# mlaprise/mfrec

Measured on NVIDIA B200. Metric: rating_updates_per_s, higher is better.
Workload: dtype f32

## Files before the change

### include/mfrec_b200.h

```cpp
#ifndef MFREC_B200_H
#define MFREC_B200_H

#include <stdint.h>

#ifdef __cplusplus
extern "C" {
#endif

#define MFREC_B200_ABI_VERSION 6

typedef enum mfrec_status {
    MFREC_OK = 0,
    MFREC_ERR_BAD_ARG = -1,
    MFREC_ERR_INDEX = -2,
    MFREC_ERR_OOM = -3,
    MFREC_ERR_CUDA = -4,
    MFREC_ERR_UNSUPPORTED = -5
} mfrec_status;

typedef struct mfrec_ctx mfrec_ctx;
typedef struct mfrec_ratings mfrec_ratings;
typedef struct mfrec_model mfrec_model;

enum { MFREC_KERNEL_LINEAR = 0,
       MFREC_KERNEL_LOGISTIC = 1    };

enum { MFREC_FUNK_WITHOUT_BIAS = 0,
       MFREC_FUNK_WITH_BIAS = 1,
       MFREC_FUNK_WITH_BIAS_DEV = 2   };

enum { MFREC_PRED_GD_RATING = 0,
       MFREC_PRED_GD_RATING_BIAS = 1,
// ... 117 lines not shown
int mfrec_bias_stats(mfrec_ctx *ctx, const int32_t *ratings_index, const double *ratings,
                     int64_t nnz, int32_t ni, int32_t nu, double K2, double K3, double *mu_out,
                     double *items_bias, double *users_bias);

int mfrec_train_als_wrmf(mfrec_ctx *ctx, int nbr_epochs, int k, double *u, double *v,
                         const int32_t *users_row, int64_t n_users_row, const int32_t *users_col,
                         const int32_t *items_row, int64_t n_items_row, const int32_t *items_col,
                         int32_t nbr_users, int32_t nbr_items, int c_pos, double reg);

int mfrec_train_als_wrmf_multi(const int32_t *devices, int n_shards, int nbr_epochs, int k,
                               double *u, double *v,
                               const int32_t *users_row, int64_t n_users_row, const int32_t *users_col,
                               const int32_t *items_row, int64_t n_items_row, const int32_t *items_col,
                               int32_t nbr_users, int32_t nbr_items, int c_pos, double reg);


int mfrec_ratings_pack(mfrec_ctx *ctx, const int32_t *ratings_index, const void *ratings,
                       int ratings_are_f32, int is_device, int64_t nnz, int32_t ni, int32_t nu,
                       const int64_t *item_degree, const mfrec_opts *opts,
                       mfrec_ratings **out);
void mfrec_ratings_destroy(mfrec_ratings *r);
int mfrec_ratings_info(const mfrec_ratings *r, int64_t info[8]);
int mfrec_ratings_quad_types(const mfrec_ratings *r, int64_t counts[4]);
int mfrec_ratings_perm(mfrec_ctx *ctx, const mfrec_ratings *r, int32_t *user_perm,
                       int32_t *item_perm);
int mfrec_ratings_order(mfrec_ctx *ctx, const mfrec_ratings *r, int64_t *order);
int mfrec_ratings_offsets(mfrec_ctx *ctx, const mfrec_ratings *r, int64_t *offsets,
                          int32_t *counts);
int mfrec_ratings_packed(mfrec_ctx *ctx, const mfrec_ratings *r, void *out);
int mfrec_ratings_copies(const mfrec_ratings *r, int32_t *vbase, int64_t counts[2]);
int mfrec_ratings_slab_items(const mfrec_ratings *r, int32_t slab, int32_t *begin, int32_t *end);

int mfrec_model_create(mfrec_ctx *ctx, const mfrec_ratings *layout, int k, int32_t ni,
                       int32_t nu, const double *u, const double *v, const double *items_bias,
                       const double *users_bias, mfrec_model **out);
int mfrec_model_read(mfrec_ctx *ctx, const mfrec_model *m, double *u, double *v,
                     double *items_bias, double *users_bias);
void mfrec_model_destroy(mfrec_model *m);
int mfrec_model_device_ptrs(const mfrec_model *m, void *ptrs[4], int64_t dims[3]);

int mfrec_sgd_epoch(mfrec_ctx *ctx, const mfrec_ratings *r, mfrec_model *m, int kernel,
                    double learning_rate, double K_users, double K_items, double K_bias,
                    int update_users, int update_items, int32_t slab, double *sq_err_out);

typedef struct mfrec_ring mfrec_ring;
int mfrec_ring_create(mfrec_ctx *ctx, const mfrec_ratings *r, mfrec_model *m, int rank, int world,
// ... 33 lines not shown
```

### mfrec_b200/_native.py

```python
import ctypes as C
import os
import threading

import numpy as np

_HERE = os.path.dirname(os.path.abspath(__file__))
LIB_PATH = os.environ.get("MFREC_B200_LIB") or os.path.join(_HERE, "libmfrec_b200.so")

OK = 0
ERR_BAD_ARG, ERR_INDEX, ERR_OOM, ERR_CUDA, ERR_UNSUPPORTED = -1, -2, -3, -4, -5

KERNEL_LINEAR, KERNEL_LOGISTIC = 0, 1
FUNK_WITHOUT_BIAS, FUNK_WITH_BIAS, FUNK_WITH_BIAS_DEV = 0, 1, 2
SCHED_STRATIFIED, SCHED_SEQUENTIAL = 0, 1
FOLD_USERS, FOLD_ITEMS = 0, 1

PREDICTORS = {
    "predict_rating": 0,
    "predict_rating_with_bias": 1,
    "predict_linear": 2,
    "predict_logistic": 3,
    "predict_linear_neg": 4,
    "predict_dot": 5,
}

EXPORTS = (
    "mfrec_abi_version", "mfrec_ctx_create", "mfrec_ctx_destroy", "mfrec_last_error",
    "mfrec_ctx_stream", "mfrec_ctx_sync", "mfrec_ctx_launch_count", "mfrec_train_kmf",
    "mfrec_train_funk", "mfrec_funk_loop_dev", "mfrec_funk_subloop", "mfrec_funk_predictor_subloop",
    "mfrec_train_funk_learned_bias", "mfrec_train_als_wrmf", "mfrec_predict_pairs", "mfrec_rmse_pairs", "mfrec_topn", "mfrec_topn_sweep",
    "mfrec_bias_stats", "mfrec_ratings_pack", "mfrec_ratings_destroy", "mfrec_ratings_info",
    "mfrec_ratings_quad_types", "mfrec_ratings_perm", "mfrec_ratings_order", "mfrec_ratings_offsets", "mfrec_ratings_packed",
    "mfrec_ratings_slab_items", "mfrec_model_create", "mfrec_model_read", "mfrec_model_destroy",
    "mfrec_model_device_ptrs", "mfrec_sgd_epoch", "mfrec_model_predict",
    "mfrec_ring_create", "mfrec_ring_destroy", "mfrec_ring_handle", "mfrec_ring_connect",
    "mfrec_ring_connect_local", "mfrec_ring_epochs", "mfrec_ring_epochs_one_device", "mfrec_ring_wait",
    "mfrec_ring_sync_model", "mfrec_model_topn", "mfrec_model_topn_sweep", "mfrec_ratings_copies",
    "mfrec_train_kmf_multi", "mfrec_fold_in_kmf", "mfrec_fold_in_funk", "mfrec_train_als_wrmf_multi",
)


class MfrecError(RuntimeError):

    def __init__(self, code, message):
        RuntimeError.__init__(self, "libmfrec_b200 error %d: %s" % (code, message))
        self.code = code


SPLIT_AUTO, SPLIT_ON, SPLIT_OFF = 0, 1, 2
STORAGE_F32, STORAGE_F16, STORAGE_BF16 = 0, 1, 2


class Opts(C.Structure):
    _fields_ = [("schedule", C.c_int32), ("row_blocks", C.c_int32), ("workers", C.c_int32),
                ("n_slabs", C.c_int32), ("keep_order", C.c_int32), ("k_hint", C.c_int32),
# ... 382 lines not shown
        _check(lib().mfrec_ratings_perm(self.ctx.handle, self._h, _ptr(up), _ptr(ip)), self.ctx.handle)
        return up, ip

    def order(self):
        out = np.zeros(self.packed_len, dtype=np.int64)
        _check(lib().mfrec_ratings_order(self.ctx.handle, self._h, _ptr(out)), self.ctx.handle)
        return out

    def offsets(self):
        off = np.zeros(self.n_buckets + 1, dtype=np.int64)
        cnt = np.zeros(self.n_buckets, dtype=np.int32)
        _check(lib().mfrec_ratings_offsets(self.ctx.handle, self._h, _ptr(off), _ptr(cnt)),
               self.ctx.handle)
        return off, cnt

    def packed(self):
        raw = np.zeros((self.packed_len, 3), dtype=np.int32)
        _check(lib().mfrec_ratings_packed(self.ctx.handle, self._h, _ptr(raw)), self.ctx.handle)
        return raw[:, 0].copy(), raw[:, 1].copy(), raw[:, 2].copy().view(np.float32)

    def quad_types(self):
        out = (C.c_int64 * 4)()
        _check(lib().mfrec_ratings_quad_types(self._h, out))
        return dict(generic=int(out[0]), chain=int(out[1]), clean=int(out[2]), independent=int(out[3]))

    def copies(self):
        vb = np.zeros(self.ni + 1, dtype=np.int32)
        cnt = (C.c_int64 * 2)()
        _check(lib().mfrec_ratings_copies(self._h, _ptr(vb), cnt))
        return vb, int(cnt[0]), int(cnt[1])

    def slab_items(self, slab):
        a, b = C.c_int32(), C.c_int32()
        _check(lib().mfrec_ratings_slab_items(self._h, C.c_int32(slab), C.byref(a), C.byref(b)))
        return a.value, b.value

    def replay_order(self, by_slab=False):
        order = self.order()
        off, cnt = self.offsets()
        B, W, G = self.B, self.W, self.G
        off = off[:-1].reshape(G, B, B, W * W)
        cnt = cnt.reshape(G, B, B, W * W)
        slabs = []
        for g in range(G):
            out = []
            for s in range(B):
                for rb in range(B):
# ... 181 lines not shown
```

### mfrec_b200/csrc/common.cuh

```cuda
#pragma once

#include <cuda_bf16.h>
#include <cuda_fp16.h>
#include <cuda_runtime.h>
#include <stdint.h>

#include <cstdarg>
#include <cstdio>
#include <future>
#include <memory>
#include <string>
#include <vector>

#include "mfrec_b200.h"

struct __align__(4) PackedRating {
    int32_t u;
    int32_t i;
    float r;
};
static_assert(sizeof(PackedRating) == 12, "rating triple must be 12 bytes");
constexpr int32_t kIdMask = 0x07ffffff;
constexpr int32_t kFlagAdjUser = 1 << 27;
constexpr int32_t kFlagStale = 1 << 28;
constexpr int32_t kFlagSameItem = 1 << 29;
constexpr int32_t kFlagPad = 1 << 30;
constexpr int kQuadShift = 28;
constexpr int kQuadGeneric = 0;
constexpr int kQuadChain = 1;
constexpr int kQuadClean = 2;
constexpr int kQuadIndep = 3;

struct mfrec_ctx {
    int device = 0;
    int sm_count = 0;
    size_t smem_optin = 0;
    size_t smem_per_sm = 0;
    int coop_launch = 0;
    cudaStream_t stream = nullptr;
    int64_t launches = 0;
    double *se_scratch = nullptr;
    size_t se_cap = 0;
    int32_t *ticks = nullptr;
    size_t ticks_cap = 0;
    cudaStream_t copy_stream = nullptr;
    cudaEvent_t values_ready = nullptr;
    struct {
        const double *u = nullptr, *v = nullptr, *ib = nullptr, *ub = nullptr;
        cudaEvent_t ready = nullptr;
    } staged;
    std::shared_future<int> values_enqueued, factors_enqueued;
    int refs = 1;
    std::shared_ptr<void> pack_host;
    std::shared_ptr<void> stager;
    std::string err;
};
void mfrec_ctx_retain(mfrec_ctx *ctx);
void mfrec_ctx_release(mfrec_ctx *ctx);

struct mfrec_ratings {
    mfrec_ctx *ctx = nullptr;
    int device = 0;
    int64_t nnz = 0;
    int32_t ni = 0, nu = 0;
    int B = 1, W = 1, G = 1;
    int storage = 0;
    int64_t n_buckets = 0;
    int64_t packed_len = 0;
    int32_t max_cb_items = 0;
    int64_t max_bucket = 0;
    float max_abs_rating = 0.f;
    int64_t quad_types[4] = {0, 0, 0, 0};
    int32_t ni_v = 0;
    int32_t n_hot = 0;
    int32_t *user_perm = nullptr;
    int32_t *item_perm = nullptr;
    int32_t *item_rows = nullptr;
    int32_t *item_vbase = nullptr;
    int32_t *vitem_src = nullptr;
    int32_t *hot_off = nullptr;
    int32_t *hot_rows = nullptr;
    int32_t *col_start = nullptr;
    PackedRating *packed = nullptr;
    int64_t *bucket_off = nullptr;
    int32_t *bucket_cnt = nullptr;
    int64_t *order = nullptr;
    std::vector<int32_t> h_row_start;
    std::vector<int32_t> h_col_start;
    std::vector<int32_t> h_vbase;
};

struct mfrec_model {
    mfrec_ctx *ctx = nullptr;
    int device = 0;
    int k = 0, kpad = 0;
// ... 22 lines not shown
            const int lu = __shfl_sync(full, level, pu < 0 ? lane : pu);
            const int li = __shfl_sync(full, level, pi < 0 ? lane : pi);
            int nl = 1;
            if (pu >= 0) nl = lu + 1;
            if (pi >= 0) nl = max(nl, li + 1);
            const bool changed = nl != level;
            level = nl;
            if (!__any_sync(full, changed)) break;
        }
    }
    lmax = __reduce_max_sync(full, live ? level : 0);
    return level;
}

__device__ __forceinline__ uint32_t smem_u32(const void *p) { return (uint32_t)__cvta_generic_to_shared(p); }
__device__ __forceinline__ void mbar_init(uint64_t *bar, uint32_t count)
{
    asm volatile("mbarrier.init.shared::cta.b64 [%0], %1;" ::"r"(smem_u32(bar)), "r"(count));
}
__device__ __forceinline__ void mbar_expect_tx(uint64_t *bar, uint32_t bytes)
{
    asm volatile("mbarrier.arrive.expect_tx.shared::cta.b64 _, [%0], %1;" ::"r"(smem_u32(bar)), "r"(bytes) : "memory");
}
__device__ __forceinline__ void mbar_wait(uint64_t *bar, uint32_t parity)
{
    asm volatile(
        "{\n"
        ".reg .pred p;\n"
        "WAIT_%=:\n"
        "mbarrier.try_wait.parity.shared::cta.b64 p, [%0], %1;\n"
        "@p bra DONE_%=;\n"
        "bra WAIT_%=;\n"
        "DONE_%=:\n"
        "}\n" ::"r"(smem_u32(bar)),
        "r"(parity)
        : "memory");
}
__device__ __forceinline__ void bulk_g2s(void *dst_smem, const void *src_gmem, uint32_t bytes, uint64_t *bar)
{
    asm volatile(
        "cp.async.bulk.shared::cluster.global.mbarrier::complete_tx::bytes [%0], [%1], %2, [%3];" ::"r"(smem_u32(dst_smem)),
        "l"(src_gmem), "r"(bytes), "r"(smem_u32(bar))
        : "memory");
}

__device__ __forceinline__ int ld_acquire_gpu(const int32_t *p)
{
// ... 136 lines not shown
```

### mfrec_b200/csrc/pack.cu

```cuda
#include <algorithm>
#include <cstring>
#include <cub/device/device_radix_sort.cuh>
#include <cub/device/device_scan.cuh>
#include <numeric>
#include <queue>

#include "common.cuh"
#include "partition.h"

namespace {

__global__ void degree_kernel(const int32_t *__restrict__ idx, int64_t nnz, int32_t ni, int32_t nu,
                              int32_t *__restrict__ deg_u, int32_t *__restrict__ deg_i,
                              int32_t *__restrict__ bad)
{
    const int64_t stride = (int64_t)gridDim.x * blockDim.x;
    for (int64_t n = (int64_t)blockIdx.x * blockDim.x + threadIdx.x; n < nnz; n += stride) {
        const int2 ui = reinterpret_cast<const int2 *>(idx)[n];
        if (ui.x < 0 || ui.x >= nu || ui.y < 0 || ui.y >= ni) {
            atomicOr(bad, 1);
            continue;
        }
        atomicAdd(&deg_u[ui.x], 1);
        atomicAdd(&deg_i[ui.y], 1);
// ... 123 lines not shown
    }
}

__global__ void max_abs_rating_kernel(const PackedRating *__restrict__ packed, int64_t n,
                                      int32_t *__restrict__ out_bits)
{
    int32_t mx = 0;
    const int64_t stride = (int64_t)gridDim.x * blockDim.x;
    for (int64_t j = (int64_t)blockIdx.x * blockDim.x + threadIdx.x; j < n; j += stride)
        mx = max(mx, __float_as_int(fabsf(packed[j].r)));
    for (int o = 16; o > 0; o >>= 1) mx = max(mx, __shfl_xor_sync(0xffffffffu, mx, o));
    if ((threadIdx.x & 31) == 0) atomicMax(out_bits, mx);
}

__global__ void fill_padding_kernel(PackedRating *__restrict__ packed, int64_t n)
{
    const int64_t stride = (int64_t)gridDim.x * blockDim.x;
    PackedRating pad;
    pad.u = 0; pad.i = kFlagPad; pad.r = 0.f;
    for (int64_t j = (int64_t)blockIdx.x * blockDim.x + threadIdx.x; j < n; j += stride) packed[j] = pad;
}

__global__ void quad_type_kernel(PackedRating *__restrict__ packed, int64_t n_quads,
                                 unsigned long long *__restrict__ type_count)
{
    const int64_t stride = (int64_t)gridDim.x * blockDim.x;
    int mine[4] = {0, 0, 0, 0};
    for (int64_t q = (int64_t)blockIdx.x * blockDim.x + threadIdx.x; q < n_quads; q += stride) {
        const int4 *src = reinterpret_cast<const int4 *>(packed + q * 4);
        const int4 a = src[0], b = src[1], c = src[2];
        const int i0 = a.y, i1 = b.x, i2 = b.w, i3 = c.z;
        const int any = i0 | i1 | i2 | i3;
        int type = kQuadGeneric;
        if (!(any & (kFlagPad | kFlagStale))) {
            const int m0 = i0 & kIdMask;
            const bool one_item = (i1 & kIdMask) == m0 && (i2 & kIdMask) == m0 && (i3 & kIdMask) == m0;
            type = (one_item && !(any & kFlagAdjUser)) ? kQuadChain : kQuadClean;
            const int m1 = i1 & kIdMask, m2 = i2 & kIdMask, m3 = i3 & kIdMask;
            if (!(any & kFlagAdjUser) && m0 != m1 && m0 != m2 && m0 != m3 && m1 != m2 && m1 != m3 && m2 != m3)
                type = kQuadIndep;
        }
        packed[q * 4].u = (a.x & kIdMask) | (type << kQuadShift);
        if (!(i0 & kFlagPad)) mine[type] += 1;
    }
#pragma unroll
    for (int t = 0; t < 4; ++t) {
        const int tot = __reduce_add_sync(0xffffffffu, mine[t]);
        if ((threadIdx.x & 31) == 0 && tot) atomicAdd(type_count + t, (unsigned long long)tot);
    }
}

__global__ void fill_i64_kernel(int64_t *p, int64_t n, int64_t v)
{
    const int64_t i = (int64_t)blockIdx.x * blockDim.x + threadIdx.x;
    if (i < n) p[i] = v;
}

int bits_for(int64_t n)
{
    int b = 1;
    while ((1ll << b) < n) ++b;
    return b;
}

__global__ void degree_key_kernel(const int32_t *__restrict__ deg, int32_t n, uint64_t seed,
                                  uint64_t *__restrict__ keys, int32_t *__restrict__ ids)
{
    const int32_t i = blockIdx.x * blockDim.x + threadIdx.x;
    if (i >= n) return;
    uint64_t x = seed ^ (uint64_t)i;
    x += 0x9e3779b97f4a7c15ull;
// ... 295 lines not shown
    DevBuf<uint32_t> vals_a, vals_b;
    MF_CUDA(ctx, keys_a.alloc(nnz, ctx->stream));
    MF_CUDA(ctx, keys_b.alloc(nnz, ctx->stream));
    MF_CUDA(ctx, vals_a.alloc(nnz, ctx->stream));
    MF_CUDA(ctx, vals_b.alloc(nnz, ctx->stream));
    cub::DoubleBuffer<uint64_t> dkeys(keys_a.p, keys_b.p);
    cub::DoubleBuffer<uint32_t> dvals(vals_a.p, vals_b.p);
    if (nnz > 0) {
        key_kernel<<<grid, 256, 0, st>>>(d_idx, nnz, R->user_perm, R->item_perm, d_ug.p, d_ig.p, R->item_vbase, kl,
                                         keys_a.p, vals_a.p);
        MF_LAUNCH_CHECK(ctx);
        size_t tmp_bytes = 0;
        const int end_bit = kl.bits_i + kl.bits_u + kl.bits_b;
        MF_CUDA(ctx, cub::DeviceRadixSort::SortPairs(nullptr, tmp_bytes, dkeys, dvals, nnz, 0, end_bit, st));
        DevBuf<char> tmp;
        MF_CUDA(ctx, tmp.alloc(tmp_bytes, ctx->stream));
        MF_CUDA(ctx, cub::DeviceRadixSort::SortPairs(tmp.p, tmp_bytes, dkeys, dvals, nnz, 0, end_bit, st));
        ctx->launches += (end_bit + 7) / 8 * 2 + 1;
        MF_CUDA(ctx, cudaStreamSynchronize(st));
    }

    tr.lap("keys + radix sort");
    DevBuf<unsigned long long> d_stats;
    MF_CUDA(ctx, d_stats.alloc(5, ctx->stream));
    MF_CUDA(ctx, cudaMemsetAsync(d_stats.p, 0, 40, st));
    int32_t *d_stats32 = reinterpret_cast<int32_t *>(d_stats.p + 4);
    const int64_t nb = R->n_buckets;
    DevBuf<int64_t> raw_cnt, pad_cnt, raw_off;
    MF_CUDA(ctx, cudaMallocAsync((void **)&R->bucket_cnt, (size_t)nb * 4, st));
    MF_CUDA(ctx, cudaMallocAsync((void **)&R->bucket_off, ((size_t)nb + 1) * 8, st));
    MF_CUDA(ctx, raw_cnt.alloc(nb + 1, ctx->stream));
    MF_CUDA(ctx, pad_cnt.alloc(nb + 1, ctx->stream));
    MF_CUDA(ctx, raw_off.alloc(nb + 1, ctx->stream));
    MF_CUDA(ctx, cudaMemsetAsync(R->bucket_cnt, 0, (size_t)nb * 4, st));
    MF_CUDA(ctx, cudaMemsetAsync(raw_cnt.p, 0, ((size_t)nb + 1) * 8, st));
    MF_CUDA(ctx, cudaMemsetAsync(pad_cnt.p, 0, ((size_t)nb + 1) * 8, st));
    if (nnz > 0) {
        bucket_hist_kernel<<<grid, 256, 0, st>>>(dkeys.Current(), nnz, kl.bits_u + kl.bits_i, R->bucket_cnt);
        MF_LAUNCH_CHECK(ctx);
    }
    pad_counts_kernel<<<(unsigned)ceil_div64(nb, 256), 256, 0, st>>>(R->bucket_cnt, nb, raw_cnt.p, pad_cnt.p,
                                                                      d_stats32 + 1);
    MF_LAUNCH_CHECK(ctx);
    {
        size_t tmp_bytes = 0;
        MF_CUDA(ctx, cub::DeviceScan::ExclusiveSum(nullptr, tmp_bytes, raw_cnt.p, raw_off.p, nb + 1, st));
        DevBuf<char> tmp;
        MF_CUDA(ctx, tmp.alloc(tmp_bytes, ctx->stream));
// ... 19 lines not shown
        const int urc = ctx->values_enqueued.get();
        ctx->values_enqueued = {};
        if (urc != MFREC_OK) return urc;
    }
    if (ctx->values_ready) {
        cudaEvent_t ev = ctx->values_ready;
        ctx->values_ready = nullptr;
        MF_CUDA(ctx, cudaStreamWaitEvent(st, ev, 0));
    }
    if (nnz > 0) {
        if (ratings_are_f32)
            gather_kernel<float><<<grid, 256, 0, st>>>(dkeys.Current(), dvals.Current(), nnz,
                                                       (const float *)d_r, kl, raw_off.p,
                                                       R->bucket_off, R->packed, R->order);
        else
            gather_kernel<double><<<grid, 256, 0, st>>>(dkeys.Current(), dvals.Current(), nnz,
                                                        (const double *)d_r, kl, raw_off.p,
                                                        R->bucket_off, R->packed, R->order);
        MF_LAUNCH_CHECK(ctx);
    }
    if (packed_len > 0) {
        hint_kernel<<<grid, 256, 0, st>>>(R->packed, packed_len);
        MF_LAUNCH_CHECK(ctx);
        quad_type_kernel<<<grid, 256, 0, st>>>(R->packed, packed_len / 4, d_stats.p);
        MF_LAUNCH_CHECK(ctx);
        max_abs_rating_kernel<<<grid, 256, 0, st>>>(R->packed, packed_len, d_stats32);
        MF_LAUNCH_CHECK(ctx);
    }
    {
        unsigned long long h_stats[5];
        MF_CUDA(ctx, cudaMemcpyAsync(h_stats, d_stats.p, 40, cudaMemcpyDeviceToHost, st));
        MF_CUDA(ctx, cudaStreamSynchronize(st));
        for (int t = 0; t < 4; ++t) R->quad_types[t] = (int64_t)h_stats[t];
        int32_t tail[2];
        memcpy(tail, &h_stats[4], 8);
        memcpy(&R->max_abs_rating, &tail[0], 4);
        R->max_bucket = tail[1];
    }
    tr.lap("gather + stats");
    guard.r = nullptr;
    *out = R;
    return MFREC_OK;
}

extern "C" int mfrec_ratings_info(const mfrec_ratings *r, int64_t info[8])
{
    if (!r || !info) return mfrec_set_error(nullptr, MFREC_ERR_BAD_ARG, "mfrec_ratings_info: NULL argument");
    info[0] = r->B;
    info[1] = r->W;
    info[2] = r->G;
    info[3] = r->max_cb_items;
    info[4] = r->nnz;
    info[5] = (int64_t)r->G * r->B;
    info[6] = r->max_bucket;
    info[7] = r->packed_len;
    return MFREC_OK;
}

extern "C" int mfrec_ratings_quad_types(const mfrec_ratings *r, int64_t counts[4])
{
    if (!r || !counts) return mfrec_set_error(nullptr, MFREC_ERR_BAD_ARG, "mfrec_ratings_quad_types: NULL argument");
    for (int t = 0; t < 4; ++t) counts[t] = r->quad_types[t];
    return MFREC_OK;
}

extern "C" int mfrec_ratings_perm(mfrec_ctx *ctx, const mfrec_ratings *r, int32_t *user_perm,
                                  int32_t *item_perm)
{
    if (!ctx || !r) return mfrec_set_error(ctx, MFREC_ERR_BAD_ARG, "mfrec_ratings_perm: NULL argument");
    MF_CUDA(ctx, cudaSetDevice(ctx->device));
    if (user_perm) MF_CUDA(ctx, cudaMemcpy(user_perm, r->user_perm, (size_t)r->nu * 4, cudaMemcpyDeviceToHost));
    if (item_perm) MF_CUDA(ctx, cudaMemcpy(item_perm, r->item_rows, (size_t)r->ni * 4, cudaMemcpyDeviceToHost));
    return MFREC_OK;
}

extern "C" int mfrec_ratings_order(mfrec_ctx *ctx, const mfrec_ratings *r, int64_t *order)
{
    if (!ctx || !r || !order) return mfrec_set_error(ctx, MFREC_ERR_BAD_ARG, "mfrec_ratings_order: NULL argument");
    if (!r->order)
        return mfrec_set_error(ctx, MFREC_ERR_BAD_ARG, "mfrec_ratings_order: pack with opts.keep_order = 1");
    MF_CUDA(ctx, cudaSetDevice(ctx->device));
    MF_CUDA(ctx, cudaMemcpy(order, r->order, (size_t)r->packed_len * 8, cudaMemcpyDeviceToHost));
    return MFREC_OK;
}

extern "C" int mfrec_ratings_offsets(mfrec_ctx *ctx, const mfrec_ratings *r, int64_t *offsets,
                                     int32_t *counts)
{
// ... 42 lines not shown
```

### mfrec_b200/csrc/sgd.cu

```cuda
#include <algorithm>
#include <cmath>
#include <cstdlib>
#include <cstring>
#include <thread>
#include <type_traits>

#include <cuda_bf16.h>
#include <cuda_fp16.h>

#include "common.cuh"
#include "fold.h"

namespace {

constexpr int kChunk = 64;
constexpr int kStages = 4;
constexpr int kDepth = 16;
constexpr int kQuadsAhead = kDepth / 4;
constexpr int kRing = kChunk * kStages;
static_assert(kChunk % 4 == 0, "chunks must be 16-byte multiples");
static_assert(4 * kDepth <= kChunk, "the prefetch cursor may run at most one chunk ahead");

struct SgdRank {
    const PackedRating *packed;
// ... 193 lines not shown
    asm volatile("mov.u64 %0, %globaltimer;" : "=l"(t));
    return t;
}

template <int E, int KERNEL, int MAXT, bool GATED, bool RING, typename PT = float>
__global__ void __launch_bounds__(MAXT, 1)
sgd_block_kernel(const SgdParams prm)
{
    constexpr int KPAD = E * 32;
    constexpr unsigned FULL = 0xffffffffu;
    extern __shared__ __align__(128) unsigned char smem_raw[];
    const int W = prm.W;
    const int warp = threadIdx.x >> 5, lane = threadIdx.x & 31;
    const int rb = RING ? (int)(blockIdx.x % (unsigned)prm.B) : (int)blockIdx.x;
    const SgdRank R = RING ? prm.ranks[blockIdx.x / (unsigned)prm.B] : prm.self;
    __shared__ int abort_s;

    float *Qs = reinterpret_cast<float *>(smem_raw);
    float *ibs = Qs + (size_t)prm.tile_rows * KPAD;
    PT *prow_all = reinterpret_cast<PT *>(ibs + ((prm.tile_rows + 3) & ~3));
    float *pbias_all = reinterpret_cast<float *>(prow_all + (size_t)W * kDepth * KPAD);
    PackedRating *ring_all = reinterpret_cast<PackedRating *>(pbias_all + (size_t)W * kDepth);
    uint64_t *bars = reinterpret_cast<uint64_t *>(ring_all + (size_t)W * kRing);
    int64_t *boff = reinterpret_cast<int64_t *>(bars + 1 + kStages * W);
    double *se_s = reinterpret_cast<double *>(boff + W * W + 2);
    volatile int32_t *phase_done = reinterpret_cast<volatile int32_t *>(se_s + W);

    PT *prow = prow_all + (size_t)warp * kDepth * KPAD;
    float *pbias = pbias_all + warp * kDepth;
    PackedRating *ring = ring_all + (size_t)warp * kRing;
    uint64_t *tile_bar = bars;
    uint64_t *my_bar = bars + 1 + kStages * warp;

    if (threadIdx.x == 0) {
        mbar_init(tile_bar, 1);
        for (int i = 0; i < kStages * W; ++i) mbar_init(bars + 1 + i, 1);
        for (int i = 0; i < W; ++i) phase_done[i] = 0;
        abort_s = 0;
        asm volatile("fence.mbarrier_init.release.cluster;" ::: "memory");
    }

    const float lr = prm.lr;
    const bool upd_u = !GATED || prm.update_users != 0, upd_i = !GATED || prm.update_items != 0;
    const float a_i = upd_i ? 1.f - prm.lr * prm.Ki : 1.f;
    const float a_u = upd_u ? 1.f - prm.lr * prm.Ku : 1.f;
    const float a_b = 1.f - prm.lr * prm.Kb;
    const unsigned long long a_i2 = pack2(a_i, a_i), a_u2 = pack2(a_u, a_u);
    const bool upd_bu = (KERNEL == MFREC_KERNEL_LINEAR) || upd_u;
    const bool upd_bi = (KERNEL == MFREC_KERNEL_LINEAR) || upd_i;
    const float fx_scale = prm.fx_scale, fx_inv = prm.fx_inv;
    constexpr uint32_t kRowBytes = KPAD * sizeof(PT);
    PT *const P_rows = reinterpret_cast<PT *>(R.P);
    PT *const P_lane = P_rows + lane * Frag<E>::V;
    uint32_t rng = 0x9e3779b9u * (blockIdx.x * 1024u + threadIdx.x + 1u);
    float *const ub_g = R.ub;
    const int64_t steps_per_epoch = (int64_t)prm.G * prm.B;

    double se = 0.0;
    uint32_t chunk_seq = 0;
    uint32_t tile_seq = 0;
// ... 18 lines not shown
        const int cs = R.col_start[cbg * W];
        const int nq = R.col_start[(cbg + 1) * W] - cs;
        const int tick_need = RING ? (int)it : epoch_rel * prm.B + s;

        const int64_t bucket_base = (((int64_t)slab * prm.B + rb) * prm.B + cbl) * W * W;
        for (int i = threadIdx.x; i <= W * W; i += blockDim.x) boff[i] = R.bucket_off[bucket_base + i];
        if (threadIdx.x == 0) {
            if (R.ticks) {
                if constexpr (RING) {
                    const unsigned long long t0 = global_ns();
                    uint32_t polls = 0;
                    while (ld_acquire_sys(R.ticks + cbg) < tick_need) {
                        __nanosleep(128);
                        if ((++polls & 1023u) == 0) {
                            if (*(volatile int32_t *)R.abort) { abort_s = 1; break; }
                            if (prm.wait_ns && global_ns() - t0 > prm.wait_ns) {
                                *(volatile int32_t *)R.abort = 1;
                                abort_s = 1;
                                break;
                            }
                        }
                    }
                } else {
                    while (ld_acquire_gpu(R.ticks + cbg) < tick_need) __nanosleep(64);
                }
                asm volatile("fence.proxy.async;" ::: "memory");
            }
            bool go = nq > 0;
            if constexpr (RING) go = go && !abort_s;
            if (go) {
                const uint32_t total = (uint32_t)nq * KPAD * 4u;
                mbar_expect_tx(tile_bar, total);
                const char *src = reinterpret_cast<const char *>(R.Q + (size_t)cs * KPAD);
                char *dst = reinterpret_cast<char *>(Qs);
                for (uint32_t o = 0; o < total; o += 32768u)
                    bulk_g2s(dst + o, src + o, min(32768u, total - o), tile_bar);
            }
        }
        __syncthreads();
        if constexpr (RING) {
            if (abort_s) break;
        }

        const int64_t S0 = boff[warp * W];
        const uint32_t slen = (uint32_t)(boff[warp * W + W] - S0);
        const uint32_t nchunks = (slen + kChunk - 1) / kChunk;
        const uint32_t nquads = slen / 4;
        const PackedRating *stream = R.packed + S0;
        const int64_t *off_w = boff + warp * W;

        constexpr uint32_t kRingQ = kRing / 4, kChunkQ = kChunk / 4;
        static_assert((kRingQ & (kRingQ - 1)) == 0 && (kChunkQ & (kChunkQ - 1)) == 0 &&
                      (kQuadsAhead & (kQuadsAhead - 1)) == 0, "ring sizes must be powers of two");
        const uint32_t base_q = (chunk_seq % kStages) * kChunkQ;
        const char *const ring_b = reinterpret_cast<const char *>(ring);
        auto quad_rec = [&](uint32_t x) { return ring_b + ((base_q + x) & (kRingQ - 1)) * 48u; };
        auto chunk_wait = [&](uint32_t c) {
            const uint32_t g = chunk_seq + c;
            mbar_wait(my_bar + (g % kStages), (g / kStages) & 1u);
        };
        auto issue_chunk = [&](uint32_t c) {
            if (lane == 0) {
                const uint32_t cnt = min((uint32_t)kChunk, slen - c * kChunk);
                const uint32_t g = chunk_seq + c;
                uint64_t *bar = my_bar + (g % kStages);
// ... 11 lines not shown
                const char *rec = quad_rec(fx);
                const uint32_t fslot0 = (fx & (kQuadsAhead - 1)) * 4;
#pragma unroll
                for (int t = 0; t < 4; ++t) {
                    const uint32_t ut = *reinterpret_cast<const uint32_t *>(rec + 12 * t) & kIdMask;
                    const PT *gsrc = row_ptr(P_lane, ut, kRowBytes);
#pragma unroll
                    for (int c = 0; c < Frag<E>::NV; ++c)
                        cp_async<Frag<E>::V * sizeof(PT)>(prow_lane + (fslot0 + t) * KPAD + c * 32 * Frag<E>::V,
                                                          gsrc + c * 32 * Frag<E>::V);
                }
                if (lane < 4) {
                    const uint32_t ul = *reinterpret_cast<const uint32_t *>(rec + 12 * lane) & kIdMask;
                    cp_async<4>(pbias + fslot0 + lane, row_ptr(ub_g, ul, 4));
                }
            }
            cp_async_commit();
        }

        if (nq > 0) {
            mbar_wait(tile_bar, tile_seq & 1u);
            tile_seq += 1;
        }
        for (int i = threadIdx.x; i < nq; i += blockDim.x) ibs[i] = __ldcg(R.ib + cs + i);
        __syncthreads();

        Frag<E> cp, cq;
#pragma unroll
        for (int e = 0; e < E; ++e) { cp.x[e] = 0.f; cq.x[e] = 0.f; }
        float cbu = 0.f, cbi = 0.f, se_f = 0.f;
        int prev_u = -1, prev_i = -1;

        auto warp_sum_fx = [&](int v) { return __reduce_add_sync(FULL, v); };
        auto dot_fx = [&](const Frag<E> &pu, const Frag<E> &q) {
            float part;
            if constexpr (E >= 2) {
                unsigned long long acc = mul2(pack2(pu.x[0], pu.x[1]), pack2(q.x[0], q.x[1]));
#pragma unroll
                for (int e = 2; e < E; e += 2)
                    acc = fma2(pack2(pu.x[e], pu.x[e + 1]), pack2(q.x[e], q.x[e + 1]), acc);
                float lo, hi;
                unpack2(acc, lo, hi);
                part = lo + hi;
            } else {
                part = pu.x[0] * q.x[0];
            }
            return __float2int_rn(part * fx_scale);
// ... 117 lines not shown
            }
            int f[4], sm[4];
#pragma unroll
            for (int t = 0; t < 4; ++t) f[t] = dot_fx(p4[t], q4[t]);
#pragma unroll
            for (int t = 0; t < 4; ++t) sm[t] = warp_sum_fx(f[t]);
#pragma unroll
            for (int t = 0; t < 4; ++t) hook(t);
#pragma unroll
            for (int t = 0; t < 4; ++t) apply(sm[t], r4[t], p4[t], b4[t], q4[t], c4[t]);
#pragma unroll
            for (int t = 0; t < 4; ++t) {
                store_q(i4[t], q4[t], c4[t]);
                store_p_row(u4[t], p4[t]);
            }
            store_bias_quad(u4, b4, 0xfu);
#pragma unroll
            for (int e = 0; e < E; ++e) { cp.x[e] = p4[3].x[e]; cq.x[e] = q4[3].x[e]; }
            cbu = b4[3];
            cbi = c4[3];
            prev_u = u4[3];
            prev_i = i4[3];
        };
        auto clean_quad = [&](uint32_t slot0, const int (&u4)[4], const int (&i4)[4], const int (&f4)[4],
                              const float (&r4)[4], auto &&hook) {
            Frag<E> p4[4];
            float b4[4];
            load_quad_p(slot0, p4, b4);
#pragma unroll
            for (int t = 0; t < 4; ++t) {
                if (f4[t] & kFlagAdjUser) {
#pragma unroll
                    for (int e = 0; e < E; ++e) p4[t].x[e] = t ? p4[t ? t - 1 : 0].x[e] : cp.x[e];
                    b4[t] = t ? b4[t ? t - 1 : 0] : cbu;
                }
                if (i4[t] != prev_i) {
                    frag_load<E>(cq, Qs + (size_t)(i4[t] - cs) * KPAD, lane);
                    cbi = ibs[i4[t] - cs];
                }
                prev_i = i4[t];
                const int isum = warp_sum_fx(dot_fx(p4[t], cq));
                hook(t);
                apply(isum, r4[t], p4[t], b4[t], cq, cbi);
                store_q(i4[t], cq, cbi);
                store_p_row(u4[t], p4[t]);
            }
            {
                uint32_t keep = 0x8u;
#pragma unroll
                for (int t = 0; t < 3; ++t) keep |= (f4[t + 1] & kFlagAdjUser) ? 0u : (1u << t);
                store_bias_quad(u4, b4, keep);
            }
#pragma unroll
            for (int e = 0; e < E; ++e) cp.x[e] = p4[3].x[e];
            cbu = b4[3];
            prev_u = u4[3];
            prev_i = i4[3];
        };

        const int32_t done_base = step * W;
        uint32_t x = 0;
        int4 na = make_int4(0, 0, 0, 0), nb = na, nc = na;
        if (nquads > 0) {
            const int4 *nsrc = reinterpret_cast<const int4 *>(quad_rec(0));
            na = nsrc[0]; nb = nsrc[1]; nc = nsrc[2];
        }
        for (int p = 0; p < W; ++p) {
            const uint32_t xe = (uint32_t)(off_w[p + 1] - S0) >> 2;
            if (p > 0) {
                const volatile int32_t *flag = phase_done + (warp + 1 == W ? 0 : warp + 1);
                if (lane == 0) {
                    while (*flag < done_base + p) __nanosleep(32);
                    __threadfence_block();
                }
                __syncwarp();
            }
            se_f = 0.f;
#pragma unroll 1
            for (; x < xe; ++x) {
                if ((x & (kChunkQ - 1)) == 0 && x != 0) {
                    const uint32_t nc = x / kChunkQ - 1 + kStages;
                    if (nc < nchunks) {
                        __syncwarp();
                        issue_chunk(nc);
                    }
                }
                const uint32_t fx = x + (kQuadsAhead - 1);
                if ((fx & (kChunkQ - 1)) == 0 && fx < nquads) chunk_wait(fx / kChunkQ);
                const char *const frec = quad_rec(min(fx, nquads - 1));
                const uint32_t fu[4] = {*reinterpret_cast<const uint32_t *>(frec) & kIdMask,
                                        *reinterpret_cast<const uint32_t *>(frec + 12) & kIdMask,
                                        *reinterpret_cast<const uint32_t *>(frec + 24) & kIdMask,
                                        *reinterpret_cast<const uint32_t *>(frec + 36) & kIdMask};
                const uint32_t fslot0 = (fx & (kQuadsAhead - 1)) * 4;
                PT *const fdst = prow_lane + fslot0 * KPAD;
                auto fetch_row = [&](int t) {
                    const PT *gsrc = row_ptr(P_lane, fu[t], kRowBytes);
#pragma unroll
                    for (int c = 0; c < Frag<E>::NV; ++c)
                        cp_async<Frag<E>::V * sizeof(PT)>(fdst + t * KPAD + c * 32 * Frag<E>::V, gsrc + c * 32 * Frag<E>::V);
                };
                cp_async_wait<kQuadsAhead - 2>();
                __syncwarp();
                const int4 a = na, b = nb, c2 = nc;
                {
                    const int4 *nsrc = reinterpret_cast<const int4 *>(quad_rec(x + 1));
                    na = nsrc[0]; nb = nsrc[1]; nc = nsrc[2];
                }
                const uint32_t slot0 = (x & (kQuadsAhead - 1)) * 4;
                const int u4[4] = {a.x & kIdMask, a.w & kIdMask, b.z & kIdMask, c2.y & kIdMask};
                const int f4[4] = {a.y, b.x, b.w, c2.z};
                const int i4[4] = {a.y & kIdMask, b.x & kIdMask, b.w & kIdMask, c2.z & kIdMask};
                const float r4[4] = {__int_as_float(a.z), __int_as_float(b.y), __int_as_float(c2.x), __int_as_float(c2.w)};
                const int qtype = (a.x >> kQuadShift) & 3;
                if (qtype == kQuadIndep) {
                    indep_quad(slot0, u4, i4, r4, fetch_row);
                } else if (qtype == kQuadChain) {
                    chain_quad(slot0, u4, i4[0], r4, fetch_row);
                } else if (qtype == kQuadClean) {
                    clean_quad(slot0, u4, i4, f4, r4, fetch_row);
                } else {
#pragma unroll
                    for (int t = 0; t < 4; ++t) {
                        if (!(f4[t] & kFlagPad)) update_one(slot0 + t, u4[t], i4[t], r4[t], (f4[t] & kFlagStale) != 0);
                        fetch_row(t);
                    }
                }
                {
                    const bool lo = (lane & 2) == 0, even = (lane & 1) == 0;
                    const uint32_t ul = lo ? (even ? fu[0] : fu[1]) : (even ? fu[2] : fu[3]);
                    if (lane < 4) cp_async<4>(pbias + fslot0 + lane, row_ptr(ub_g, ul, 4));
                }
                cp_async_commit();
            }
            se += (double)se_f;
            prev_i = -1;
            __syncwarp();
            if (lane == 0) {
                __threadfence_block();
                phase_done[warp] = done_base + p + 1;
            }
        }
        cp_async_wait<0>();
        chunk_seq += nchunks;
        chunks_issued = false;
        int ns = s + 1, nt = t_slab;
        if (ns == prm.B) {
            ns = 0;
            nt = t_slab + 1 == prm.G ? 0 : t_slab + 1;
        }
        if (it + 1 < prm.it_end) {
            int nslab = R.rank + nt;
            if (nslab >= prm.G) nslab -= prm.G;
            int ncbl = rb + ns;
            if (ncbl >= prm.B) ncbl -= prm.B;
            const int64_t nbase = ((((int64_t)nslab * prm.B + rb) * prm.B + ncbl) * W + warp) * W;
            const int64_t nS0 = __ldg(R.bucket_off + nbase);
            const uint32_t nslen = (uint32_t)(__ldg(R.bucket_off + nbase + W) - nS0);
            const uint32_t nn = min((nslen + kChunk - 1) / kChunk, (uint32_t)kStages);
            if (lane == 0) {
                for (uint32_t c = 0; c < nn; ++c) {
                    const uint32_t cnt = min((uint32_t)kChunk, nslen - c * kChunk);
                    const uint32_t g = chunk_seq + c;
                    uint64_t *bar = my_bar + (g % kStages);
                    mbar_expect_tx(bar, cnt * 12u);
                    bulk_g2s(ring + (g % kStages) * kChunk, R.packed + nS0 + (size_t)c * kChunk, cnt * 12u, bar);
                }
            }
            chunks_issued = true;
        }
        __syncthreads();
        const bool to_peer = RING && s + 1 == prm.B && prm.world > 1;
        {
            const int nvec = nq * KPAD / 4;
            float4 *dst = reinterpret_cast<float4 *>((to_peer ? R.peer_Q : R.Q) + (size_t)cs * KPAD);
            float *dst_b = (to_peer ? R.peer_ib : R.ib) + cs;
            const float4 *srcv = reinterpret_cast<const float4 *>(Qs);
            float chk = 0.f;
            for (int i = threadIdx.x; i < nvec; i += blockDim.x) {
                const float4 t = srcv[i];
                chk = fmaf(0.f, t.x, fmaf(0.f, t.y, fmaf(0.f, t.z, fmaf(0.f, t.w, chk))));
                dst[i] = t;
            }
            for (int i = threadIdx.x; i < nq; i += blockDim.x) {
                chk = fmaf(0.f, ibs[i], chk);
                dst_b[i] = ibs[i];
            }
            if (__any_sync(FULL, chk != chk)) se = NAN;
        }
        const bool epoch_ends = in_epoch + 1 == (int)steps_per_epoch || it + 1 == prm.it_end;
        if (epoch_ends) {
            if (lane == 0) se_s[warp] = se;
            se = 0.0;
        }
        if (R.ticks) {
            if constexpr (RING) {
                if (to_peer) {
                    __threadfence_system();
                    __syncthreads();
                    if (threadIdx.x == 0) st_release_sys(R.peer_ticks + cbg, tick_need + 1);
                } else {
// ... 248 lines not shown
            double fb = linear ? fbias[c] : __ldg(fbias + c);
            const double e2 = SIDE == MFREC_FOLD_USERS
                ? kmf_rating(kernel, dim, lr, K_users, K_items, K_bias, r, other, mine, fb, b, 1, 0)
                : kmf_rating(kernel, dim, lr, K_users, K_items, K_bias, r, mine, other, b, fb, 0, 1);
            if (linear) fbias[c] = fb;
            se = __dadd_rn(se, e2);
        }
        rmse[(size_t)j * nbr_epochs + epoch] = sqrt(se / (double)(e - a));
    }
    if (SMEM)
        for (int f = 0; f < dim; ++f) grow[f] = mine.ld(f);
    tbias[row] = b;
}

}

size_t mfrec_sgd_smem_bytes(int tile_rows, int kpad, int W, int p_elem_bytes)
{
    size_t b = (size_t)tile_rows * kpad * 4;
    b += (size_t)((tile_rows + 3) & ~3) * 4;
    b += (size_t)W * kDepth * kpad * p_elem_bytes;
    b += (size_t)W * kDepth * 4;
    b += (size_t)W * kRing * sizeof(PackedRating);
    b += (size_t)(1 + kStages * W) * 8;
    b += (size_t)(W * W + 2) * 8;
    b += (size_t)W * 8;
    b += (size_t)((W + 3) & ~3) * 4;
    return b + 384;
}

namespace {

template <int E>
int launch_sgd(mfrec_ctx *ctx, int kernel, SgdParams &prm, size_t smem, bool cooperative, int grid, bool ring,
               int p_kind)
{
    const bool wide = prm.W > 8;
    const bool gated = !(prm.update_users && prm.update_items);
    void (*fn)(const SgdParams) = nullptr;
    const bool mid = prm.W > 8 && prm.W <= 12 && !gated;
#define MF_PICK(K)                                                                                     \
    fn = mid ? sgd_block_kernel<E, K, 384, false, false>                                                \
       : wide ? (gated ? sgd_block_kernel<E, K, 512, true, false> : sgd_block_kernel<E, K, 512, false, false>) \
              : (gated ? sgd_block_kernel<E, K, 256, true, false> : sgd_block_kernel<E, K, 256, false, false>)
#define MF_PICK_RING(K) \
    fn = mid ? sgd_block_kernel<E, K, 384, false, true>                                                  \
       : wide ? sgd_block_kernel<E, K, 512, false, true> : sgd_block_kernel<E, K, 256, false, true>
    if (p_kind != MFREC_STORAGE_F32) {
        if constexpr (E >= 2) {
            if (ring || gated || prm.W > 12)
// ... 764 lines not shown
```

Baseline: 6.290 billion.

## Use mbarriers for intra-block phase handoff and skip forwarding in clean quads

Replaces the volatile phase_done flag spin-wait between warps with a per-phase mbarrier array (arrive/wait with parity), dropping nanosleep polling. Packing now tags clean quads that have no adjacent-user dependencies with a new flag bit, so the SGD kernel takes a specialised clean_quad path with no forwarding checks and an unconditional bias store. It also prefetches the first item-bias value before the tile wait, removes nanosleep from the ticks spin, and unrolls the Q write-back loop. Adds shared memory for W*W barriers, and busy-spinning without sleep may contend for issue slots with working warps.

```diff
diff --git a/include/mfrec_b200.h b/include/mfrec_b200.h
--- a/include/mfrec_b200.h
+++ b/include/mfrec_b200.h
@@ -7,7 +7,7 @@
 extern "C" {
 #endif
 
-#define MFREC_B200_ABI_VERSION 6
+#define MFREC_B200_ABI_VERSION 7
 
 typedef enum mfrec_status {
     MFREC_OK = 0,
@@ -171,6 +171,7 @@
 void mfrec_ratings_destroy(mfrec_ratings *r);
 int mfrec_ratings_info(const mfrec_ratings *r, int64_t info[8]);
 int mfrec_ratings_quad_types(const mfrec_ratings *r, int64_t counts[4]);
+int mfrec_ratings_clean_no_forward(const mfrec_ratings *r, int64_t *count);
 int mfrec_ratings_perm(mfrec_ctx *ctx, const mfrec_ratings *r, int32_t *user_perm,
                        int32_t *item_perm);
 int mfrec_ratings_order(mfrec_ctx *ctx, const mfrec_ratings *r, int64_t *order);
diff --git a/mfrec_b200/_native.py b/mfrec_b200/_native.py
--- a/mfrec_b200/_native.py
+++ b/mfrec_b200/_native.py
@@ -30,7 +30,7 @@
     "mfrec_train_funk", "mfrec_funk_loop_dev", "mfrec_funk_subloop", "mfrec_funk_predictor_subloop",
     "mfrec_train_funk_learned_bias", "mfrec_train_als_wrmf", "mfrec_predict_pairs", "mfrec_rmse_pairs", "mfrec_topn", "mfrec_topn_sweep",
     "mfrec_bias_stats", "mfrec_ratings_pack", "mfrec_ratings_destroy", "mfrec_ratings_info",
-    "mfrec_ratings_quad_types", "mfrec_ratings_perm", "mfrec_ratings_order", "mfrec_ratings_offsets", "mfrec_ratings_packed",
+    "mfrec_ratings_quad_types", "mfrec_ratings_clean_no_forward", "mfrec_ratings_perm", "mfrec_ratings_order", "mfrec_ratings_offsets", "mfrec_ratings_packed",
     "mfrec_ratings_slab_items", "mfrec_model_create", "mfrec_model_read", "mfrec_model_destroy",
     "mfrec_model_device_ptrs", "mfrec_sgd_epoch", "mfrec_model_predict",
     "mfrec_ring_create", "mfrec_ring_destroy", "mfrec_ring_handle", "mfrec_ring_connect",
@@ -459,7 +459,10 @@
     def quad_types(self):
         out = (C.c_int64 * 4)()
         _check(lib().mfrec_ratings_quad_types(self._h, out))
-        return dict(generic=int(out[0]), chain=int(out[1]), clean=int(out[2]), independent=int(out[3]))
+        nf = C.c_int64(0)
+        _check(lib().mfrec_ratings_clean_no_forward(self._h, C.byref(nf)))
+        return dict(generic=int(out[0]), chain=int(out[1]), clean=int(out[2]), independent=int(out[3]),
+                    clean_no_forward=int(nf.value))
 
     def copies(self):
         vb = np.zeros(self.ni + 1, dtype=np.int32)
diff --git a/mfrec_b200/csrc/common.cuh b/mfrec_b200/csrc/common.cuh
--- a/mfrec_b200/csrc/common.cuh
+++ b/mfrec_b200/csrc/common.cuh
@@ -30,6 +30,7 @@
 constexpr int kQuadChain = 1;
 constexpr int kQuadClean = 2;
 constexpr int kQuadIndep = 3;
+constexpr int32_t kQuadNoFwd = 1 << 27;
 
 struct mfrec_ctx {
     int device = 0;
@@ -70,7 +71,7 @@
     int32_t max_cb_items = 0;
     int64_t max_bucket = 0;
     float max_abs_rating = 0.f;
-    int64_t quad_types[4] = {0, 0, 0, 0};
+    int64_t quad_types[5] = {0, 0, 0, 0, 0};
     int32_t ni_v = 0;
     int32_t n_hot = 0;
     int32_t *user_perm = nullptr;
@@ -139,7 +140,11 @@
 {
     asm volatile("mbarrier.arrive.expect_tx.shared::cta.b64 _, [%0], %1;" ::"r"(smem_u32(bar)), "r"(bytes) : "memory");
 }
-__device__ __forceinline__ void mbar_wait(uint64_t *bar, uint32_t parity)
+__device__ __forceinline__ void mbar_arrive(uint64_t *bar)
+{
+    asm volatile("mbarrier.arrive.release.cta.shared::cta.b64 _, [%0];" ::"r"(smem_u32(bar)) : "memory");
+}
+__device__ __forceinline__ void mbar_wait(const uint64_t *bar, uint32_t parity)
 {
     asm volatile(
         "{\n"
diff --git a/mfrec_b200/csrc/pack.cu b/mfrec_b200/csrc/pack.cu
--- a/mfrec_b200/csrc/pack.cu
+++ b/mfrec_b200/csrc/pack.cu
@@ -169,10 +169,10 @@
 }
 
 __global__ void quad_type_kernel(PackedRating *__restrict__ packed, int64_t n_quads,
-                                 unsigned long long *__restrict__ type_count)
-{
-    const int64_t stride = (int64_t)gridDim.x * blockDim.x;
-    int mine[4] = {0, 0, 0, 0};
+                                 unsigned long long *__restrict__ type_count, unsigned long long *__restrict__ no_fwd_count)
+{
+    const int64_t stride = (int64_t)gridDim.x * blockDim.x;
+    int mine[5] = {0, 0, 0, 0, 0};
     for (int64_t q = (int64_t)blockIdx.x * blockDim.x + threadIdx.x; q < n_quads; q += stride) {
         const int4 *src = reinterpret_cast<const int4 *>(packed + q * 4);
         const int4 a = src[0], b = src[1], c = src[2];
@@ -187,13 +187,17 @@
             if (!(any & kFlagAdjUser) && m0 != m1 && m0 != m2 && m0 != m3 && m1 != m2 && m1 != m3 && m2 != m3)
                 type = kQuadIndep;
         }
-        packed[q * 4].u = (a.x & kIdMask) | (type << kQuadShift);
-        if (!(i0 & kFlagPad)) mine[type] += 1;
+        const bool no_fwd = type == kQuadClean && !(any & kFlagAdjUser);
+        packed[q * 4].u = (a.x & kIdMask) | (type << kQuadShift) | (no_fwd ? kQuadNoFwd : 0);
+        if (!(i0 & kFlagPad)) {
+            mine[type] += 1;
+            mine[4] += no_fwd ? 1 : 0;
+        }
     }
 #pragma unroll
-    for (int t = 0; t < 4; ++t) {
+    for (int t = 0; t < 5; ++t) {
         const int tot = __reduce_add_sync(0xffffffffu, mine[t]);
-        if ((threadIdx.x & 31) == 0 && tot) atomicAdd(type_count + t, (unsigned long long)tot);
+        if ((threadIdx.x & 31) == 0 && tot) atomicAdd(t < 4 ? type_count + t : no_fwd_count, (unsigned long long)tot);
     }
 }
 
@@ -535,8 +539,8 @@
 
     tr.lap("keys + radix sort");
     DevBuf<unsigned long long> d_stats;
-    MF_CUDA(ctx, d_stats.alloc(5, ctx->stream));
-    MF_CUDA(ctx, cudaMemsetAsync(d_stats.p, 0, 40, st));
+    MF_CUDA(ctx, d_stats.alloc(6, ctx->stream));
+    MF_CUDA(ctx, cudaMemsetAsync(d_stats.p, 0, 48, st));
     int32_t *d_stats32 = reinterpret_cast<int32_t *>(d_stats.p + 4);
     const int64_t nb = R->n_buckets;
     DevBuf<int64_t> raw_cnt, pad_cnt, raw_off;
@@ -602,16 +606,17 @@
     if (packed_len > 0) {
         hint_kernel<<<grid, 256, 0, st>>>(R->packed, packed_len);
         MF_LAUNCH_CHECK(ctx);
-        quad_type_kernel<<<grid, 256, 0, st>>>(R->packed, packed_len / 4, d_stats.p);
+        quad_type_kernel<<<grid, 256, 0, st>>>(R->packed, packed_len / 4, d_stats.p, d_stats.p + 5);
         MF_LAUNCH_CHECK(ctx);
         max_abs_rating_kernel<<<grid, 256, 0, st>>>(R->packed, packed_len, d_stats32);
         MF_LAUNCH_CHECK(ctx);
     }
     {
-        unsigned long long h_stats[5];
-        MF_CUDA(ctx, cudaMemcpyAsync(h_stats, d_stats.p, 40, cudaMemcpyDeviceToHost, st));
+        unsigned long long h_stats[6];
+        MF_CUDA(ctx, cudaMemcpyAsync(h_stats, d_stats.p, 48, cudaMemcpyDeviceToHost, st));
         MF_CUDA(ctx, cudaStreamSynchronize(st));
         for (int t = 0; t < 4; ++t) R->quad_types[t] = (int64_t)h_stats[t];
+        R->quad_types[4] = (int64_t)h_stats[5];
         int32_t tail[2];
         memcpy(tail, &h_stats[4], 8);
         memcpy(&R->max_abs_rating, &tail[0], 4);
@@ -644,6 +649,13 @@
     return MFREC_OK;
 }
 
+extern "C" int mfrec_ratings_clean_no_forward(const mfrec_ratings *r, int64_t *count)
+{
+    if (!r || !count) return mfrec_set_error(nullptr, MFREC_ERR_BAD_ARG, "mfrec_ratings_clean_no_forward: NULL argument");
+    *count = r->quad_types[4];
+    return MFREC_OK;
+}
+
 extern "C" int mfrec_ratings_perm(mfrec_ctx *ctx, const mfrec_ratings *r, int32_t *user_perm,
                                   int32_t *item_perm)
 {
diff --git a/mfrec_b200/csrc/sgd.cu b/mfrec_b200/csrc/sgd.cu
--- a/mfrec_b200/csrc/sgd.cu
+++ b/mfrec_b200/csrc/sgd.cu
@@ -239,9 +239,9 @@
     float *pbias_all = reinterpret_cast<float *>(prow_all + (size_t)W * kDepth * KPAD);
     PackedRating *ring_all = reinterpret_cast<PackedRating *>(pbias_all + (size_t)W * kDepth);
     uint64_t *bars = reinterpret_cast<uint64_t *>(ring_all + (size_t)W * kRing);
-    int64_t *boff = reinterpret_cast<int64_t *>(bars + 1 + kStages * W);
+    uint64_t *phase_bar = bars + 1 + kStages * W;
+    int64_t *boff = reinterpret_cast<int64_t *>(phase_bar + W * W);
     double *se_s = reinterpret_cast<double *>(boff + W * W + 2);
-    volatile int32_t *phase_done = reinterpret_cast<volatile int32_t *>(se_s + W);
 
     PT *prow = prow_all + (size_t)warp * kDepth * KPAD;
     float *pbias = pbias_all + warp * kDepth;
@@ -251,8 +251,7 @@
 
     if (threadIdx.x == 0) {
         mbar_init(tile_bar, 1);
-        for (int i = 0; i < kStages * W; ++i) mbar_init(bars + 1 + i, 1);
-        for (int i = 0; i < W; ++i) phase_done[i] = 0;
+        for (int i = 0; i < kStages * W + W * W; ++i) mbar_init(bars + 1 + i, 1);
         abort_s = 0;
         asm volatile("fence.mbarrier_init.release.cluster;" ::: "memory");
     }
@@ -317,7 +316,8 @@
                         }
                     }
                 } else {
-                    while (ld_acquire_gpu(R.ticks + cbg) < tick_need) __nanosleep(64);
+                    while (ld_acquire_gpu(R.ticks + cbg) < tick_need) {
+                    }
                 }
                 asm volatile("fence.proxy.async;" ::: "memory");
             }
@@ -336,6 +336,7 @@
         if constexpr (RING) {
             if (abort_s) break;
         }
+        const float ib_first = (int)threadIdx.x < nq ? __ldcg(R.ib + cs + threadIdx.x) : 0.f;
 
         const int64_t S0 = boff[warp * W];
         const uint32_t slen = (uint32_t)(boff[warp * W + W] - S0);
@@ -393,7 +394,8 @@
             mbar_wait(tile_bar, tile_seq & 1u);
             tile_seq += 1;
         }
-        for (int i = threadIdx.x; i < nq; i += blockDim.x) ibs[i] = __ldcg(R.ib + cs + i);
+        if ((int)threadIdx.x < nq) ibs[threadIdx.x] = ib_first;
+        for (int i = threadIdx.x + blockDim.x; i < nq; i += blockDim.x) ibs[i] = __ldcg(R.ib + cs + i);
         __syncthreads();
 
         Frag<E> cp, cq;
@@ -557,14 +559,15 @@
             prev_u = u4[3];
             prev_i = i4[3];
         };
-        auto clean_quad = [&](uint32_t slot0, const int (&u4)[4], const int (&i4)[4], const int (&f4)[4],
+        auto clean_quad = [&](auto fwd, uint32_t slot0, const int (&u4)[4], const int (&i4)[4], const int (&f4)[4],
                               const float (&r4)[4], auto &&hook) {
+            constexpr bool kFwd = decltype(fwd)::value;
             Frag<E> p4[4];
             float b4[4];
             load_quad_p(slot0, p4, b4);
 #pragma unroll
             for (int t = 0; t < 4; ++t) {
-                if (f4[t] & kFlagAdjUser) {
+                if (kFwd && (f4[t] & kFlagAdjUser)) {
 #pragma unroll
                     for (int e = 0; e < E; ++e) p4[t].x[e] = t ? p4[t ? t - 1 : 0].x[e] : cp.x[e];
                     b4[t] = t ? b4[t ? t - 1 : 0] : cbu;
@@ -580,11 +583,13 @@
                 store_q(i4[t], cq, cbi);
                 store_p_row(u4[t], p4[t]);
             }
-            {
+            if constexpr (kFwd) {
                 uint32_t keep = 0x8u;
 #pragma unroll
                 for (int t = 0; t < 3; ++t) keep |= (f4[t + 1] & kFlagAdjUser) ? 0u : (1u << t);
                 store_bias_quad(u4, b4, keep);
+            } else {
+                store_bias_quad(u4, b4, 0xfu);
             }
 #pragma unroll
             for (int e = 0; e < E; ++e) cp.x[e] = p4[3].x[e];
@@ -593,7 +598,8 @@
             prev_i = i4[3];
         };
 
-        const int32_t done_base = step * W;
+        const uint32_t phase_parity = (uint32_t)step & 1u;
+        const uint64_t *const next_bar = phase_bar + (warp + 1 == W ? 0 : warp + 1) * W;
         uint32_t x = 0;
         int4 na = make_int4(0, 0, 0, 0), nb = na, nc = na;
         if (nquads > 0) {
@@ -602,14 +608,7 @@
         }
         for (int p = 0; p < W; ++p) {
             const uint32_t xe = (uint32_t)(off_w[p + 1] - S0) >> 2;
-            if (p > 0) {
-                const volatile int32_t *flag = phase_done + (warp + 1 == W ? 0 : warp + 1);
-                if (lane == 0) {
-                    while (*flag < done_base + p) __nanosleep(32);
-                    __threadfence_block();
-                }
-                __syncwarp();
-            }
+            if (p > 0) mbar_wait(next_bar + (p - 1), phase_parity);
             se_f = 0.f;
 #pragma unroll 1
             for (; x < xe; ++x) {
@@ -653,7 +652,10 @@
                 } else if (qtype == kQuadChain) {
                     chain_quad(slot0, u4, i4[0], r4, fetch_row);
                 } else if (qtype == kQuadClean) {
-                    clean_quad(slot0, u4, i4, f4, r4, fetch_row);
+                    if (a.x & kQuadNoFwd)
+                        clean_quad(std::false_type{}, slot0, u4, i4, f4, r4, fetch_row);
+                    else
+                        clean_quad(std::true_type{}, slot0, u4, i4, f4, r4, fetch_row);
                 } else {
 #pragma unroll
                     for (int t = 0; t < 4; ++t) {
@@ -670,10 +672,9 @@
             }
             se += (double)se_f;
             prev_i = -1;
-            __syncwarp();
-            if (lane == 0) {
-                __threadfence_block();
-                phase_done[warp] = done_base + p + 1;
+            if (p + 1 < W) {
+                __syncwarp();
+                if (lane == 0) mbar_arrive(phase_bar + warp * W + p);
             }
         }
         cp_async_wait<0>();
@@ -712,6 +713,7 @@
             float *dst_b = (to_peer ? R.peer_ib : R.ib) + cs;
             const float4 *srcv = reinterpret_cast<const float4 *>(Qs);
             float chk = 0.f;
+#pragma unroll 4
             for (int i = threadIdx.x; i < nvec; i += blockDim.x) {
                 const float4 t = srcv[i];
                 chk = fmaf(0.f, t.x, fmaf(0.f, t.y, fmaf(0.f, t.z, fmaf(0.f, t.w, chk))));
@@ -1006,10 +1008,9 @@
     b += (size_t)W * kDepth * kpad * p_elem_bytes;
     b += (size_t)W * kDepth * 4;
     b += (size_t)W * kRing * sizeof(PackedRating);
-    b += (size_t)(1 + kStages * W) * 8;
+    b += (size_t)(1 + kStages * W + W * W) * 8;
     b += (size_t)(W * W + 2) * 8;
     b += (size_t)W * 8;
-    b += (size_t)((W + 3) & ~3) * 4;
     return b + 384;
 }
 
```

After: 6.344 billion, median of 6. About the same (+0.9%).
